# MishaLaskin/vqvae

Hardware: NVIDIA H100
Metric: images/sec VQVAE fwd (enc+VQ+dec) (higher is better)
Workload: dtype tf32

## Files before the change

### vqvae_b200/csrc/vq_backward.cu

```cuda
#include "common.cuh"

namespace {

__global__ void vq_backward_kernel(const float *__restrict__ g_zq, const float *__restrict__ g_loss, const float *__restrict__ z,
                                   const float *__restrict__ E, const long long *__restrict__ idx, long long N, int K, int D,
                                   float beta, float *__restrict__ dz, float *__restrict__ dE) {
    const int d4 = D / 4;
    const long long total = N * d4;
    const float gl = g_loss ? __ldg(g_loss) : 0.f;
    const float c1 = gl * 2.0f / ((float)N * (float)D), c2 = c1 * beta;
    for (long long i = (long long)blockIdx.x * blockDim.x + threadIdx.x; i < total; i += (long long)gridDim.x * blockDim.x) {
        const long long row = i / d4;
        const int c = (int)(i - row * d4);
        long long k = idx[row];
        k = k < 0 ? 0 : (k >= K ? K - 1 : k);
        const float4 zv = __ldg(reinterpret_cast<const float4 *>(z) + i);
        const float4 ev = __ldg(reinterpret_cast<const float4 *>(E + (size_t)k * D) + c);
        float4 g = g_zq ? __ldg(reinterpret_cast<const float4 *>(g_zq) + i) : make_float4(0.f, 0.f, 0.f, 0.f);
        const float4 df = make_float4(zv.x - ev.x, zv.y - ev.y, zv.z - ev.z, zv.w - ev.w);
        g.x = fmaf(c1, df.x, g.x); g.y = fmaf(c1, df.y, g.y); g.z = fmaf(c1, df.z, g.z); g.w = fmaf(c1, df.w, g.w);
        reinterpret_cast<float4 *>(dz)[i] = g;
        float *de = dE + (size_t)k * D + 4 * c;
        atomicAdd(de + 0, -c2 * df.x); atomicAdd(de + 1, -c2 * df.y); atomicAdd(de + 2, -c2 * df.z); atomicAdd(de + 3, -c2 * df.w);
    }
}

}

extern "C" int vqb_vq_backward_f32(const float *g_zq, const float *g_loss, const float *z, const float *codebook,
                                   const int64_t *idx, int64_t N, int K, int D, float beta, float *dz, float *dE, void *stream) {
    if (!z || !codebook || !idx || !dz || !dE) return VQB_ERR_BAD_ARG;
    if (N <= 0 || K <= 0 || D <= 0) return VQB_ERR_BAD_ARG;
    if (D % 4 != 0) return VQB_ERR_UNSUPPORTED;
    const uintptr_t al = reinterpret_cast<uintptr_t>(z) | reinterpret_cast<uintptr_t>(codebook) | reinterpret_cast<uintptr_t>(dz) |
                         reinterpret_cast<uintptr_t>(dE) | reinterpret_cast<uintptr_t>(g_zq);
    if (al & 15) return VQB_ERR_ALIGNMENT;
    cudaStream_t s = (cudaStream_t)stream;
    cudaError_t e = cudaMemsetAsync(dE, 0, sizeof(float) * (size_t)K * D, s);
    if (e != cudaSuccess) return (int)e;
    const long long total = N * (D / 4);
    long long blocks = (total + 255) / 256;
    int dev = 0, sms = 132;
    cudaGetDevice(&dev);
    cudaDeviceGetAttribute(&sms, cudaDevAttrMultiProcessorCount, dev);
    if (blocks > (long long)sms * 16) blocks = (long long)sms * 16;
    vq_backward_kernel<<<(unsigned)blocks, 256, 0, s>>>(g_zq, g_loss, z, codebook, reinterpret_cast<const long long *>(idx), N, K, D, beta,
                                                        dz, dE);
    VQB_COUNT_LAUNCH(1);
    return vqb_cuda_status(cudaGetLastError());
}
```

### vqvae_b200/csrc/wgconv.cu

```cuda
#include "ptx.cuh"
#include "bf16_common.cuh"
#include "wgconv.h"
#include "wgmma.cuh"

namespace {

constexpr int WG_THREADS = 384;
constexpr int WG_MAX_STAGES = 8;
constexpr int A_BYTES = 128 * 128;

struct WgParams {
    const float *bias;
    const void *skip;
    void *out;
    int B, ncols, mid_cols;
    int BW, BH, BN, tiles_x, tiles_y;
    int in_step, out_step, stages;
    int relu, out_bf16;
    int OHg[4], OWg[4], out_py[4], out_px[4], nsteps[4];
    long long out_sn, out_sh, out_sw, out_sc;
    int4 steps[4][WG_MAX_STEPS];
    const void *tail_w;
    const float *tail_bias;
    float *tail_out;
    int tail_cout, tail_relu;
};

constexpr int SC_N = 64;
constexpr int SC_BBYTES = SC_N * 128;

template <bool BF16>
__device__ __forceinline__ void gather_shuffle_weight(uint32_t wres, const void *w, int Cin, int Cout, int nc, int t) {
    const size_t row_bytes = (size_t)Cin * (BF16 ? 2 : 4);
    for (int i = t; i < nc * SC_N * 8; i += 256) {
        const int j = i & 7, r = (i >> 3) % SC_N, c = i / (8 * SC_N);
        const int ph = r >> 4, k = (r >> 2) & 3, co = r & 3;
        const int tap = ((k >> 1) + (ph >> 1)) * 3 + (k & 1) + (ph & 1);
        uint4 v = make_uint4(0u, 0u, 0u, 0u);
        if (co < Cout)
            v = __ldg(reinterpret_cast<const uint4 *>(reinterpret_cast<const unsigned char *>(w) +
                      (size_t)(tap * 16 + ph * Cout + co) * row_bytes + c * 128 + j * 16));
        const uint32_t dst = wres + (uint32_t)(c * SC_BBYTES + r * 128 + ((j ^ (r & 7)) << 4));
        asm volatile("st.shared.v4.b32 [%0], {%1, %2, %3, %4};" ::"r"(dst), "r"(v.x), "r"(v.y), "r"(v.z), "r"(v.w) : "memory");
    }
    ptx::fence_proxy_async();
}

template <int N>
__device__ __forceinline__ void store_tile(const WgParams &p, const float *acc, int ph, int wgi, int gx0, int gy0, int n0,
                                           const void *skip, int relu) {
    const int warp = (threadIdx.x >> 5) & 3, lane = threadIdx.x & 31;
    const int cq = 2 * (lane & 3);
#pragma unroll
    for (int h = 0; h < 2; ++h) {
        const int row = wgi * 64 + warp * 16 + (lane >> 2) + 8 * h;
        const int bw = row % p.BW, bh = (row / p.BW) % p.BH, bn = row / (p.BW * p.BH);
        const int gx = gx0 + bw, gy = gy0 + bh, n = n0 + bn;
        if (gx >= p.OWg[ph] || gy >= p.OHg[ph] || n >= p.B) continue;
        const long long ob = (long long)n * p.out_sn + (long long)(gy * p.out_step + p.out_py[ph]) * p.out_sh +
                             (long long)(gx * p.out_step + p.out_px[ph]) * p.out_sw;
#pragma unroll
        for (int j = 0; j < N / 8; ++j) {
            const int c = 8 * j + cq;
            if (c >= p.ncols) continue;
            float v0 = acc[4 * j + 2 * h], v1 = acc[4 * j + 2 * h + 1];
            if (p.bias) { v0 += __ldg(p.bias + c); v1 += __ldg(p.bias + c + 1); }
            if (p.out_bf16) {
                if (skip) {
                    const __nv_bfloat162 sk = *reinterpret_cast<const __nv_bfloat162 *>(
                        reinterpret_cast<const __nv_bfloat16 *>(skip) + ob + c);
                    v0 += __bfloat162float(sk.x); v1 += __bfloat162float(sk.y);
                }
                if (relu) { v0 = fmaxf(v0, 0.f); v1 = fmaxf(v1, 0.f); }
                *reinterpret_cast<uint32_t *>(reinterpret_cast<__nv_bfloat16 *>(p.out) + ob + c) = pack_bf16(v0, v1);
            } else {
                if (skip) {
                    const float2 sk = *reinterpret_cast<const float2 *>(reinterpret_cast<const float *>(skip) + ob + c);
                    v0 += sk.x; v1 += sk.y;
                }
                if (relu) { v0 = fmaxf(v0, 0.f); v1 = fmaxf(v1, 0.f); }
                *reinterpret_cast<float2 *>(reinterpret_cast<float *>(p.out) + ob + c) = make_float2(v0, v1);
            }
        }
    }
}

template <bool BF16, int N>
__host__ __device__ constexpr int chain_chunks() { return BF16 ? 1 : (N >= 32 ? N / 32 : 1); }

constexpr int TAIL_PHASE_ROWS = 4 * 128;

template <bool BF16, int N, int N2, bool TAIL = false>
__global__ void __launch_bounds__(WG_THREADS, 1)
wgconv_kernel(const __grid_constant__ CUtensorMap tma_in, const __grid_constant__ CUtensorMap tma_w,
              const __grid_constant__ CUtensorMap tma_w2, const __grid_constant__ WgParams p) {
    static_assert(!TAIL || (!BF16 && N == SC_N && N2 == 0), "TAIL: TF32, 64 channels of h, no second GEMM");
    extern __shared__ unsigned char smem_raw[];
    const uint32_t raw = ptx::smem_u32(smem_raw);
    const uint32_t sbase = (raw + 1023u) & ~1023u;
    constexpr int STAGE = A_BYTES + N * 128;
    constexpr int KC2 = chain_chunks<BF16, N>();
    constexpr int HCHUNK = TAIL_PHASE_ROWS * 128;
    const int S = p.stages;
    const uint32_t mid = sbase + (uint32_t)(S * STAGE);
    const uint32_t w2s = mid + (uint32_t)(KC2 * (TAIL ? HCHUNK : A_BYTES));
    const uint32_t bars = mid + (N2 > 0 ? (uint32_t)(KC2 * (A_BYTES + N2 * 128))
                                 : TAIL ? (uint32_t)(KC2 * (HCHUNK + SC_BBYTES)) : 0u);
    auto full = [&](int s) { return bars + 8u * s; };
    auto empty = [&](int s) { return bars + 8u * (WG_MAX_STAGES + s); };
    const uint32_t w2bar = bars + 8u * (2 * WG_MAX_STAGES);

    const int tid = threadIdx.x, warp = tid >> 5, lane = tid & 31;
    const int ph0 = TAIL ? 0 : blockIdx.y, nph = TAIL ? 4 : 1;
    int tile = blockIdx.x;
    const int tx = tile % p.tiles_x; tile /= p.tiles_x;
    const int ty = tile % p.tiles_y; tile /= p.tiles_y;
    const int gx0 = tx * p.BW, gy0 = ty * p.BH, n0 = tile * p.BN;

    if (tid == 0) {
        for (int s = 0; s < S; ++s) { ptx::mbar_init(full(s), 1); ptx::mbar_init(empty(s), 2); }
        ptx::mbar_init(w2bar, 1);
        ptx::fence_mbar_init();
    }
    if (tid == 32) {
        ptx::prefetch_tmap(&tma_in);
        ptx::prefetch_tmap(&tma_w);
        if (N2 > 0) ptx::prefetch_tmap(&tma_w2);
    }
    __syncthreads();
    pdl_launch_dependents();

    if (warp == 0) {
        if constexpr (N2 > 0) {
            if (lane == 0) {
                constexpr int ck = BF16 ? 64 : 32;
                ptx::mbar_expect_tx(w2bar, (uint32_t)(KC2 * N2 * 128));
                for (int c = 0; c < KC2; ++c) ptx::tma_load_2d(w2s + (uint32_t)(c * N2 * 128), &tma_w2, w2bar, c * ck, 0);
            }
        }
        pdl_wait();
        if (lane == 0) {
            int g = 0;
            for (int ph = ph0; ph < ph0 + nph; ++ph)
                for (int i = 0; i < p.nsteps[ph]; ++i, ++g) {
                    const int s = g % S;
                    if (g >= S) ptx::mbar_wait(empty(s), (uint32_t)((g / S - 1) & 1));
                    const int4 st = p.steps[ph][i];
                    const uint32_t dst = sbase + (uint32_t)(s * STAGE);
                    ptx::mbar_expect_tx(full(s), (uint32_t)STAGE);
                    ptx::tma_load_4d(dst, &tma_in, full(s), st.x, gx0 * p.in_step + st.y, gy0 * p.in_step + st.z, n0);
                    ptx::tma_load_2d(dst + A_BYTES, &tma_w, full(s), st.x, st.w);
                }
        }
        return;
    }
    if (warp < 4) return;

    if constexpr (TAIL) gather_shuffle_weight<false>(w2s, p.tail_w, N, p.tail_cout, KC2, tid - 128);
    pdl_wait();
    const int wgi = (warp >> 2) - 1;
    float acc[N / 2];
    int g = 0;
    for (int ph = ph0; ph < ph0 + nph; ++ph) {
#pragma unroll
        for (int i = 0; i < N / 2; ++i) acc[i] = 0.f;
        for (int i = 0; i < p.nsteps[ph]; ++i, ++g) {
            const int s = g % S;
            ptx::mbar_wait(full(s), (uint32_t)((g / S) & 1));
            const uint32_t a = sbase + (uint32_t)(s * STAGE) + (uint32_t)(wgi * 64 * 128), b = sbase + (uint32_t)(s * STAGE) + A_BYTES;
            wg::fence();
#pragma unroll
            for (int kk = 0; kk < 4; ++kk) wg::mma<BF16, N>(acc, wg::desc_sw128(a + 32u * kk), wg::desc_sw128(b + 32u * kk), 1u);
            wg::commit();
            wg::wait<0>();
            wg::fence_regs<N>(acc);
            if ((warp & 3) == 0 && lane == 0) ptx::mbar_arrive(empty(s));
        }
        if constexpr (TAIL) {
            const int wl = warp & 3, cq = 2 * (lane & 3);
#pragma unroll
            for (int h = 0; h < 2; ++h) {
                const int row = wgi * 64 + wl * 16 + (lane >> 2) + 8 * h;
                const int bw = row % p.BW, bh = (row / p.BW) % p.BH, bn = row / (p.BW * p.BH);
                const int hr = (bn * 2 * p.BH + 2 * bh + p.out_py[ph]) * 2 * p.BW + 2 * bw + p.out_px[ph];
                const bool live = gx0 + bw < p.OWg[ph] && gy0 + bh < p.OHg[ph] && n0 + bn < p.B;
                float *o = reinterpret_cast<float *>(p.out) + (long long)(n0 + bn) * p.out_sn +
                           (long long)((gy0 + bh) * p.out_step + p.out_py[ph]) * p.out_sh +
                           (long long)((gx0 + bw) * p.out_step + p.out_px[ph]) * p.out_sw;
#pragma unroll
                for (int j = 0; j < N / 8; ++j) {
                    const int c = 8 * j + cq;
                    float v0 = acc[4 * j + 2 * h], v1 = acc[4 * j + 2 * h + 1];
                    if (p.bias) { v0 += __ldg(p.bias + c); v1 += __ldg(p.bias + c + 1); }
                    if (p.relu) { v0 = fmaxf(v0, 0.f); v1 = fmaxf(v1, 0.f); }
                    const uint32_t addr = mid + (uint32_t)((c >> 5) * HCHUNK + hr * 128 + ((((c & 31) >> 2) ^ (hr & 7)) << 4) + (c & 3) * 4);
                    asm volatile("st.shared.v2.f32 [%0], {%1, %2};" ::"r"(addr), "f"(v0), "f"(v1) : "memory");
                    if (p.out && live) *reinterpret_cast<float2 *>(o + c) = make_float2(v0, v1);
                }
            }
        }
    }

    if constexpr (TAIL) {
        ptx::fence_proxy_async();
        ptx::named_bar_sync(1, 256);
        const int wl = warp & 3, cq = 2 * (lane & 3);
        for (int blk = 4 * wgi; blk < 4 * wgi + 4; ++blk) {
            float y[SC_N / 2];
#pragma unroll
            for (int i = 0; i < SC_N / 2; ++i) y[i] = 0.f;
            wg::fence();
#pragma unroll
            for (int c = 0; c < KC2; ++c) {
                const uint32_t a = mid + (uint32_t)(c * HCHUNK + blk * 64 * 128), b = w2s + (uint32_t)(c * SC_BBYTES);
#pragma unroll
                for (int kk = 0; kk < 4; ++kk) wg::mma<false, SC_N>(y, wg::desc_sw128(a + 32u * kk), wg::desc_sw128(b + 32u * kk), 1u);
            }
            wg::commit();
            wg::wait<0>();
            wg::fence_regs<SC_N>(y);
            ptx::named_bar_sync(2 + wgi, 128);
#pragma unroll
            for (int h = 0; h < 2; ++h) {
                const int q = blk * 64 + wl * 16 + (lane >> 2) + 8 * h;
#pragma unroll
                for (int j = 0; j < SC_N / 8; ++j) {
                    const int c = 8 * j + cq;
                    const uint32_t addr = mid + (uint32_t)((c >> 5) * HCHUNK + q * 128 + (((c & 31) + 2 * q) & 31) * 4);
                    asm volatile("st.shared.v2.f32 [%0], {%1, %2};" ::"r"(addr), "f"(y[4 * j + 2 * h]), "f"(y[4 * j + 2 * h + 1]) : "memory");
                }
            }
        }
        ptx::named_bar_sync(1, 256);
        const int H = p.OHg[0], W = p.OWg[0];
        const int lw = __ffs(4 * p.BW) - 1, lh = __ffs(4 * p.BH) - 1, Cout = p.tail_cout;
        const float *const ys = reinterpret_cast<const float *>(smem_raw + (mid - raw));
        auto yat = [&](int q, int col) {
            return ys[(col >> 5) * (HCHUNK / 4) + q * 32 + (((col & 31) + 2 * q) & 31)];
        };
        const int total = (p.BN * Cout) << (lw + lh);
        for (int e = tid - 128; e < total; e += 256) {
            const int ox = e & (4 * p.BW - 1), oy = (e >> lw) & (4 * p.BH - 1), co = (e >> (lw + lh)) % Cout;
            const int bn = (e >> (lw + lh)) / Cout;
            if (ox >= 4 * W || oy >= 4 * H || n0 + bn >= p.B) continue;
            const int gy = oy >> 1, py = oy & 1, gx = ox >> 1, px = ox & 1;
            const int base = bn * 4 * p.BH * p.BW, col = (py * 2 + px) * 16 + co;
            float t[4];
#pragma unroll
            for (int k = 0; k < 4; ++k) {
                const int hy = gy + (k >> 1) + py - 1, hx = gx + (k & 1) + px - 1;
                t[k] = hy >= 0 && hy < 2 * H && hx >= 0 && hx < 2 * W ? yat(base + hy * 2 * p.BW + hx, col + 4 * k) : 0.f;
            }
            float v = t[0];
            v += t[1];
            v += t[2];
            v += t[3];
            v += p.tail_bias ? __ldg(p.tail_bias + co) : 0.f;
            if (p.tail_relu) v = fmaxf(v, 0.f);
            p.tail_out[(long long)(n0 + bn) * Cout * 16 * H * W + (long long)co * 16 * H * W + oy * 4 * W + ox] = v;
        }
    } else if constexpr (N2 == 0) {
        store_tile<N>(p, acc, ph0, wgi, gx0, gy0, n0, p.skip, p.relu);
    } else {
        const int wl = warp & 3, cq = 2 * (lane & 3);
#pragma unroll
        for (int h = 0; h < 2; ++h) {
            const int row = wgi * 64 + wl * 16 + (lane >> 2) + 8 * h;
            const uint32_t rb = mid + (uint32_t)(row * 128);
            if constexpr (BF16) {
#pragma unroll
                for (int j = 0; j < 8; ++j) {
                    const int c = 8 * j + cq;
                    float v0 = 0.f, v1 = 0.f;
                    if (j < N / 8 && c < p.mid_cols) { v0 = fmaxf(acc[4 * j + 2 * h], 0.f); v1 = fmaxf(acc[4 * j + 2 * h + 1], 0.f); }
                    const uint32_t addr = rb + (uint32_t)(((j ^ (row & 7)) << 4) + cq * 2);
                    asm volatile("st.shared.b32 [%0], %1;" ::"r"(addr), "r"(pack_bf16(v0, v1)) : "memory");
                }
            } else {
#pragma unroll
                for (int j = 0; j < N / 8; ++j) {
                    const int c = 8 * j + cq, piece = (c & 31) >> 2;
                    const float v0 = fmaxf(acc[4 * j + 2 * h], 0.f), v1 = fmaxf(acc[4 * j + 2 * h + 1], 0.f);
                    const uint32_t addr = rb + (uint32_t)((c >> 5) * A_BYTES) + (uint32_t)(((piece ^ (row & 7)) << 4) + (c & 3) * 4);
                    asm volatile("st.shared.v2.f32 [%0], {%1, %2};" ::"r"(addr), "f"(v0), "f"(v1) : "memory");
                }
            }
        }
        ptx::fence_proxy_async();
        ptx::named_bar_sync(1 + wgi, 128);
        ptx::mbar_wait(w2bar, 0);
        float acc2[N2 > 0 ? N2 / 2 : 1];
#pragma unroll
        for (int i = 0; i < N2 / 2; ++i) acc2[i] = 0.f;
        wg::fence();
#pragma unroll
        for (int c = 0; c < KC2; ++c) {
            const uint32_t a = mid + (uint32_t)(c * A_BYTES + wgi * 64 * 128), b = w2s + (uint32_t)(c * N2 * 128);
#pragma unroll
            for (int kk = 0; kk < 4; ++kk)
                wg::mma<BF16, N2>(acc2, wg::desc_sw128(a + 32u * kk), wg::desc_sw128(b + 32u * kk), 1u);
        }
        wg::commit();
        wg::wait<0>();
        wg::fence_regs<N2>(acc2);
        store_tile<N2>(p, acc2, ph0, wgi, gx0, gy0, n0, p.skip, p.relu);
    }
}

int pow2_ceil(int x) {
    int p = 1;
    while (p < x) p <<= 1;
    return p;
}

typedef void (*wg_fn)(CUtensorMap, CUtensorMap, CUtensorMap, WgParams);

template <bool BF16, int N2>
wg_fn pick_n(int N) {
    switch (N) {
        case 16: return wgconv_kernel<BF16, 16, N2>;
        case 32: return wgconv_kernel<BF16, 32, N2>;
        case 64: return wgconv_kernel<BF16, 64, N2>;
        case 128: return wgconv_kernel<BF16, 128, N2>;
        case 256: return N2 == 0 ? wgconv_kernel<BF16, 256, 0> : nullptr;
        default: return nullptr;
    }
}

wg_fn pick(int bf16, int N, int N2) {
    if (!bf16) {
        switch (N2) {
            case 0: return pick_n<false, 0>(N);
            case 64: return (N == 32 || N == 64) ? pick_n<false, 64>(N) : nullptr;
            case 128: return (N == 32 || N == 64) ? pick_n<false, 128>(N) : nullptr;
            default: return nullptr;
        }
    }
    switch (N2) {
        case 0: return pick_n<true, 0>(N);
        case 64: return N <= 64 ? pick_n<true, 64>(N) : nullptr;
        case 128: return N <= 64 ? pick_n<true, 128>(N) : nullptr;
        default: return nullptr;
    }
}

}

int wg_gemm_cols(int ncols) {
    for (int n : {16, 32, 64, 128, 256})
        if (ncols <= n) return n;
    return 0;
}

int launch_wgconv(const WgLaunch &L, cudaStream_t s) {
    if (L.nph < 1 || L.nph > 4 || wg_gemm_cols(L.N) != L.N || L.ncols > L.N) return VQB_ERR_UNSUPPORTED;
    const bool tail = L.tail_out != nullptr;
    if (tail && (L.bf16 || L.N != SC_N || L.ncols != SC_N || L.N2 != 0 || L.nph != 4 || L.out_step != 2 ||
                 L.tail_cout < 1 || L.tail_cout > 4))
        return VQB_ERR_UNSUPPORTED;
    const wg_fn fn = tail ? wgconv_kernel<false, SC_N, 0, true> : pick(L.bf16, L.N, L.N2);
    if (!fn) return VQB_ERR_UNSUPPORTED;
    const int esz = L.bf16 ? 2 : 4, ck = 128 / esz;
    if (L.Cin % ck != 0 || L.w_inner % ck != 0) return VQB_ERR_UNSUPPORTED;
    if (L.out_sc != 1) return VQB_ERR_UNSUPPORTED;
    WgParams q;
    memset(&q, 0, sizeof(q));
    q.bias = L.bias; q.skip = L.skip; q.out = L.out;
    q.B = L.B; q.ncols = L.ncols; q.mid_cols = L.ncols;
    q.in_step = L.in_step; q.out_step = L.out_step;
    q.relu = L.relu; q.out_bf16 = L.out_bf16;
    q.out_sn = L.out_sn; q.out_sh = L.out_sh; q.out_sw = L.out_sw; q.out_sc = L.out_sc;
    q.tail_w = L.tail_w; q.tail_bias = L.tail_bias; q.tail_out = L.tail_out; q.tail_cout = L.tail_cout;
    q.tail_relu = L.tail_relu;
    int maxw = 0, maxh = 0, maxk = 1;
    for (int i = 0; i < L.nph; ++i) {
        if (L.nsteps[i] > WG_MAX_STEPS) return VQB_ERR_UNSUPPORTED;
        q.OHg[i] = L.OHg[i]; q.OWg[i] = L.OWg[i]; q.out_py[i] = L.out_py[i]; q.out_px[i] = L.out_px[i];
        q.nsteps[i] = L.nsteps[i];
        for (int t = 0; t < L.nsteps[i]; ++t) {
            const WgStep &st = L.steps[i][t];
            q.steps[i][t] = make_int4(st.c0, st.dx, st.dy, st.w_row);
        }
        if (L.OWg[i] > maxw) maxw = L.OWg[i];
        if (L.OHg[i] > maxh) maxh = L.OHg[i];
        if (L.nsteps[i] > maxk) maxk = L.nsteps[i];
    }
    if (maxw <= 0 || maxh <= 0) return 0;
    q.BW = pow2_ceil(maxw) < 16 ? pow2_ceil(maxw) : 16;
    q.BH = pow2_ceil(maxh) < 128 / q.BW ? pow2_ceil(maxh) : 128 / q.BW;
    q.BN = 128 / (q.BW * q.BH);
    q.tiles_x = (maxw + q.BW - 1) / q.BW;
    q.tiles_y = (maxh + q.BH - 1) / q.BH;
    const long long tiles_n = (L.B + q.BN - 1) / q.BN;
    if (tail) {
        if (q.tiles_x != 1 || q.tiles_y != 1) return VQB_ERR_UNSUPPORTED;
        for (int i = 0; i < 4; ++i)
            if (L.OHg[i] != maxh || L.OWg[i] != maxw) return VQB_ERR_UNSUPPORTED;
    }

    const CUtensorMapDataType dt = L.bf16 ? CU_TENSOR_MAP_DATA_TYPE_BFLOAT16 : CU_TENSOR_MAP_DATA_TYPE_FLOAT32;
    CUtensorMap tin, tw, tw2;
    const uint64_t dims[4] = {(uint64_t)L.Cin, (uint64_t)L.W, (uint64_t)L.H, (uint64_t)L.B};
    const uint64_t strides[3] = {(uint64_t)L.Cin * esz, (uint64_t)L.W * L.Cin * esz, (uint64_t)L.H * L.W * L.Cin * esz};
    const uint32_t box[4] = {(uint32_t)ck, (uint32_t)(q.BW * L.in_step), (uint32_t)(q.BH * L.in_step), (uint32_t)q.BN};
    const uint32_t es[4] = {1u, (uint32_t)L.in_step, (uint32_t)L.in_step, 1u};
    int rc = vqb_encode_tmap_4d(&tin, dt, L.in, dims, strides, box, es, CU_TENSOR_MAP_SWIZZLE_128B);
    if (rc) return rc;
    rc = vqb_encode_tmap_2d(&tw, dt, L.w, (uint64_t)L.w_inner, (uint64_t)L.w_rows, (uint64_t)L.w_inner * esz, (uint32_t)ck,
                            (uint32_t)L.N, CU_TENSOR_MAP_SWIZZLE_128B);
    if (rc) return rc;
    tw2 = tw;
    int kc2 = 0;
    if (L.N2 > 0) {
        if (L.ncols > 64 || L.w2_inner % ck != 0) return VQB_ERR_UNSUPPORTED;
        if (!L.bf16 && L.ncols != L.N) return VQB_ERR_UNSUPPORTED;
        kc2 = L.bf16 ? 1 : L.N / 32;
        q.mid_cols = L.ncols; q.ncols = L.N2;
        rc = vqb_encode_tmap_2d(&tw2, dt, L.w2, (uint64_t)L.w2_inner, (uint64_t)L.w2_rows, (uint64_t)L.w2_inner * esz, (uint32_t)ck,
                                (uint32_t)L.N2, CU_TENSOR_MAP_SWIZZLE_128B);
        if (rc) return rc;
    }
    const long long grid = (long long)q.tiles_x * q.tiles_y * tiles_n;
    if (grid <= 0 || grid > 0x7fffffffLL) return VQB_ERR_UNSUPPORTED;
    const int stage = A_BYTES + L.N * 128;
    const int fixed = (tail ? (SC_N / 32) * (TAIL_PHASE_ROWS * 128 + SC_BBYTES) : kc2 * (A_BYTES + L.N2 * 128)) +
                      8 * (2 * WG_MAX_STAGES + 1) + 1024;
    auto ring = [&](int budget) {
        const int st = (budget - fixed) / stage;
        return st > WG_MAX_STAGES ? WG_MAX_STAGES : st > maxk ? maxk : st;
    };
    int stages = ring(220 * 1024);
    if (stages < 1) return VQB_ERR_UNSUPPORTED;
    static bool attr_set[64] = {false};
    const int slot = tail ? 24 : (L.bf16 ? 32 : 0) + (L.N2 == 128 ? 16 : L.N2 == 64 ? 8 : 0) + (L.N == 16 ? 0 : L.N == 32 ? 1 : L.N == 64 ? 2 : L.N == 128 ? 3 : 4);
    if (!attr_set[slot]) {
        cudaError_t e = cudaFuncSetAttribute(fn, cudaFuncAttributeMaxDynamicSharedMemorySize, 220 * 1024);
        if (e != cudaSuccess) return (int)e;
        attr_set[slot] = true;
    }
    int dev = 0, sms = 132;
    cudaGetDevice(&dev);
    cudaDeviceGetAttribute(&sms, cudaDevAttrMultiProcessorCount, dev);
    const int shared = ring(113 * 1024);
    if (!tail && grid * L.nph > sms && shared >= (maxk < 3 ? maxk : 3) && shared < stages) {
        int per_sm = 0;
        if (cudaOccupancyMaxActiveBlocksPerMultiprocessor(&per_sm, fn, WG_THREADS, (size_t)(shared * stage + fixed)) ==
                cudaSuccess && per_sm >= 2)
            stages = shared;
    }
    q.stages = stages;
    const int smem = stages * stage + fixed;
    if (cudaError_t le = vqb_launch(fn, dim3((unsigned)grid, tail ? 1u : (unsigned)L.nph), dim3(WG_THREADS), (size_t)smem, s,
                                    tin, tw, tw2, q))
        return (int)le;
    VQB_COUNT_LAUNCH(1);
    return vqb_cuda_status(cudaGetLastError());
}

static bool set_phase(WgLaunch &L, int i, const ConvPhase &ph, int rows_per_tap, bool chunk_outer) {
    const int ck = L.bf16 ? 64 : 32, nc = L.Cin / ck;
    if (ph.ntaps * nc > WG_MAX_STEPS) return false;
    L.in_step = ph.in_step; L.out_step = ph.out_step;
    L.OHg[i] = ph.OHg; L.OWg[i] = ph.OWg; L.out_py[i] = ph.out_py; L.out_px[i] = ph.out_px;
    int n = 0;
    for (int a = 0; a < (chunk_outer ? nc : ph.ntaps); ++a)
        for (int b = 0; b < (chunk_outer ? ph.ntaps : nc); ++b) {
            const int t = chunk_outer ? b : a, c0 = (chunk_outer ? a : b) * ck;
            L.steps[i][n++] = WgStep{c0, ph.tap_dx[t], ph.tap_dy[t], ph.tap_w[t] * rows_per_tap};
        }
    L.nsteps[i] = n;
    return true;
}

static ConvPhase taps3x3(int H, int W) {
    ConvPhase ph;
    conv_phase(conv_geom(3, 3, 1, 1, 0, H, W), 0, ph);
    return ph;
}

bool conv_tc_supported(const ConvLaunch &p) {
    const bool in_nhwc = p.in_sc == 1 && p.in_sw == p.Cin;
    const bool out_nhwc = p.out_sc == 1 && p.out_sw == p.Cout;
    return in_nhwc && out_nhwc && p.Cin % 32 == 0 && p.Cout % 16 == 0 && p.Cout >= 16 && p.Cout <= 256 &&
           (reinterpret_cast<uintptr_t>(p.in) & 15) == 0 && (reinterpret_cast<uintptr_t>(p.out) & 15) == 0 &&
           (p.skip == nullptr || (reinterpret_cast<uintptr_t>(p.skip) & 15) == 0);
}

int launch_conv_tc(WgLaunch &L, const ConvPhase *ph, int nph, int total_taps, bool chunk_outer, cudaStream_t s) {
    if (nph < 1 || nph > 4) return VQB_ERR_UNSUPPORTED;
    L.w_rows = (long long)total_taps * L.ncols; L.w_inner = L.Cin;
    L.N = wg_gemm_cols(L.ncols);
    L.nph = nph;
    for (int i = 0; i < nph; ++i)
        if (!set_phase(L, i, ph[i], L.ncols, chunk_outer)) return VQB_ERR_UNSUPPORTED;
    return launch_wgconv(L, s);
}

constexpr int RS_MID = 32;
constexpr int RS_N = 3 * RS_MID;
constexpr int RS_WBYTES = RS_N * 128;
constexpr int RS_YS = RS_N + 8;
constexpr int RS_MAX_STAGES = 4;
constexpr int TAIL_N = 64;

struct RsParams {
    float *out;
    const float *head_bias, *tail_bias;
    int B, H, W, BW, BH, BN, napps, relu, stages;
    int head_steps, head_stages, tail;
    int4 head[WG_MAX_STEPS];
};

template <int C>
__global__ void __launch_bounds__(WG_THREADS, 1)
res_scatter_kernel(const __grid_constant__ CUtensorMap tma_in, const __grid_constant__ CUtensorMap tma_w1,
                   const __grid_constant__ CUtensorMap tma_w2, const __grid_constant__ CUtensorMap tma_hw,
                   const __grid_constant__ CUtensorMap tma_tw, const __grid_constant__ RsParams p) {
    constexpr int NC = C / 32;
    constexpr int HSTAGE = A_BYTES + C * 128;
    extern __shared__ unsigned char smem_raw[];
    const uint32_t raw = ptx::smem_u32(smem_raw);
    const uint32_t act = (raw + 1023u) & ~1023u;
    const uint32_t ring = act + (uint32_t)(NC * A_BYTES);
    const uint32_t mid = ring + (uint32_t)(p.stages * RS_WBYTES);
    const uint32_t ysm = mid + (uint32_t)A_BYTES;
    const uint32_t w2s = ysm + (uint32_t)(128 * RS_YS * 4);
    const uint32_t bars = w2s + (uint32_t)(C * 128);
    float *const Y = reinterpret_cast<float *>(smem_raw + (ysm - raw));
    auto full = [&](int s) { return bars + 8u * s; };
    auto empty = [&](int s) { return bars + 8u * (RS_MAX_STAGES + s); };
    auto hfull = [&](int s) { return bars + 8u * (2 * RS_MAX_STAGES + s); };
    auto hempty = [&](int s) { return bars + 8u * (3 * RS_MAX_STAGES + s); };
    const uint32_t abar = bars + 8u * (4 * RS_MAX_STAGES), w2bar = abar + 8u, tbar = abar + 16u;
    const int S = p.stages, HS = p.head_stages, nh = p.head_steps;
    const int total = p.napps * 3 * NC;
    const int n0 = blockIdx.x * p.BN;

    const int tid = threadIdx.x, warp = tid >> 5, lane = tid & 31;
    if (tid == 0) {
        for (int s = 0; s < S; ++s) { ptx::mbar_init(full(s), 1); ptx::mbar_init(empty(s), 2); }
        for (int s = 0; s < HS; ++s) { ptx::mbar_init(hfull(s), 1); ptx::mbar_init(hempty(s), 2); }
        ptx::mbar_init(abar, 1);
        ptx::mbar_init(w2bar, 1);
        ptx::mbar_init(tbar, 1);
        ptx::fence_mbar_init();
    }
    if (tid == 32) {
        ptx::prefetch_tmap(&tma_in);
        ptx::prefetch_tmap(&tma_w1);
        ptx::prefetch_tmap(&tma_w2);
        if (nh) ptx::prefetch_tmap(&tma_hw);
        if (p.tail) ptx::prefetch_tmap(&tma_tw);
    }
    __syncthreads();
    pdl_launch_dependents();

    if (warp == 0) {
        auto load_w1 = [&](int g) {
            const int s = g % S;
            ptx::mbar_expect_tx(full(s), (uint32_t)RS_WBYTES);
            ptx::tma_load_2d(ring + (uint32_t)(s * RS_WBYTES), &tma_w1, full(s), (g % NC) * 32, ((g / NC) % 3) * RS_N);
        };
        auto load_weights = [&] {
            ptx::mbar_expect_tx(w2bar, (uint32_t)(C * 128));
            ptx::tma_load_2d(w2s, &tma_w2, w2bar, 0, 0);
            for (int g = 0; g < S; ++g) load_w1(g);
        };
        if (lane == 0 && !nh) load_weights();
        pdl_wait();
        if (lane == 0) {
            if (nh) {
                for (int i = 0; i < nh; ++i) {
                    const int s = i % HS;
                    if (i >= HS) ptx::mbar_wait(hempty(s), (uint32_t)((i / HS - 1) & 1));
                    const int4 st = p.head[i];
                    const uint32_t dst = ring + (uint32_t)(s * HSTAGE);
                    ptx::mbar_expect_tx(hfull(s), (uint32_t)HSTAGE);
                    ptx::tma_load_4d(dst, &tma_in, hfull(s), st.x, st.y, st.z, n0);
                    ptx::tma_load_2d(dst + A_BYTES, &tma_hw, hfull(s), st.x, st.w);
                }
                for (int i = nh > HS ? nh - HS : 0; i < nh; ++i) ptx::mbar_wait(hempty(i % HS), (uint32_t)((i / HS) & 1));
                load_weights();
            } else {
                ptx::mbar_expect_tx(abar, (uint32_t)(NC * A_BYTES));
                for (int c = 0; c < NC; ++c) ptx::tma_load_4d(act + (uint32_t)(c * A_BYTES), &tma_in, abar, c * 32, 0, 0, n0);
            }
            for (int g = S; g < total; ++g) {
                ptx::mbar_wait(empty(g % S), (uint32_t)((g / S - 1) & 1));
                load_w1(g);
            }
            if (p.tail) {
                for (int g = total - S; g < total; ++g) ptx::mbar_wait(empty(g % S), (uint32_t)((g / S) & 1));
                ptx::mbar_expect_tx(tbar, (uint32_t)(NC * TAIL_N * 128));
                for (int c = 0; c < NC; ++c) ptx::tma_load_2d(ring + (uint32_t)(c * TAIL_N * 128), &tma_tw, tbar, c * 32, 0);
            }
        }
        return;
    }
    if (warp < 4) return;

    pdl_wait();
    const int wgi = (warp >> 2) - 1, wl = warp & 3, cw = warp - 4, cq = 2 * (lane & 3);
    const int lbw = __ffs(p.BW) - 1, lbh = __ffs(p.BH) - 1;
    auto act_addr = [&](int row, int c) {
        return act + (uint32_t)((c >> 5) * A_BYTES + row * 128 + ((((c & 31) >> 2) ^ (row & 7)) << 4) + (c & 3) * 4);
    };
    auto live_row = [&](int row) {
        const int bw = row & (p.BW - 1), bh = (row >> lbw) & (p.BH - 1), bn = row >> (lbw + lbh);
        return bw < p.W && bh < p.H && n0 + bn < p.B;
    };
    if (nh) {
        float acc[C / 2];
#pragma unroll
        for (int i = 0; i < C / 2; ++i) acc[i] = 0.f;
        for (int i = 0; i < nh; ++i) {
            const int s = i % HS;
            ptx::mbar_wait(hfull(s), (uint32_t)((i / HS) & 1));
            const uint32_t a = ring + (uint32_t)(s * HSTAGE + wgi * 64 * 128), b = ring + (uint32_t)(s * HSTAGE + A_BYTES);
            wg::fence();
#pragma unroll
            for (int kk = 0; kk < 4; ++kk) wg::mma<false, C>(acc, wg::desc_sw128(a + 32u * kk), wg::desc_sw128(b + 32u * kk), 1u);
            wg::commit();
            wg::wait<0>();
            wg::fence_regs<C>(acc);
            if (wl == 0 && lane == 0) ptx::mbar_arrive(hempty(s));
        }
#pragma unroll
        for (int h = 0; h < 2; ++h) {
            const int row = wgi * 64 + wl * 16 + (lane >> 2) + 8 * h;
            const bool live = live_row(row);
#pragma unroll
            for (int j = 0; j < C / 8; ++j) {
                const int c = 8 * j + cq;
                float v0 = acc[4 * j + 2 * h], v1 = acc[4 * j + 2 * h + 1];
                if (p.head_bias) { v0 += __ldg(p.head_bias + c); v1 += __ldg(p.head_bias + c + 1); }
                v0 = fmaxf(v0, 0.f); v1 = fmaxf(v1, 0.f);
                if (!live) { v0 = 0.f; v1 = 0.f; }
                asm volatile("st.shared.v2.f32 [%0], {%1, %2};" ::"r"(act_addr(row, c)), "f"(v0), "f"(v1) : "memory");
            }
        }
        ptx::fence_proxy_async();
        ptx::named_bar_sync(2 + wgi, 128);
    } else {
        ptx::mbar_wait(abar, 0);
    }
    int g = 0;
    for (int app = 0; app < p.napps; ++app) {
        const bool last = app + 1 == p.napps;
        float m[16];
#pragma unroll
        for (int i = 0; i < 16; ++i) m[i] = 0.f;
#pragma unroll 1
        for (int r = 0; r < 3; ++r) {
            float acc[RS_N / 2];
            for (int c = 0; c < NC; ++c, ++g) {
                const int s = g % S;
                ptx::mbar_wait(full(s), (uint32_t)((g / S) & 1));
                const uint32_t a = act + (uint32_t)(c * A_BYTES + wgi * 64 * 128), b = ring + (uint32_t)(s * RS_WBYTES);
                wg::fence();
#pragma unroll
                for (int kk = 0; kk < 4; ++kk) wg::mma<false, RS_N>(acc, wg::desc_sw128(a + 32u * kk), wg::desc_sw128(b + 32u * kk), (c | kk) != 0);
                wg::commit();
                wg::wait<0>();
                wg::fence_regs<RS_N>(acc);
                if (wl == 0 && lane == 0) ptx::mbar_arrive(empty(s));
            }
            ptx::named_bar_sync(1, 256);
#pragma unroll
            for (int h = 0; h < 2; ++h) {
                float *yr = Y + (wgi * 64 + wl * 16 + (lane >> 2) + 8 * h) * RS_YS + cq;
#pragma unroll
                for (int j = 0; j < RS_N / 8; ++j)
                    *reinterpret_cast<float2 *>(yr + 8 * j) = make_float2(acc[4 * j + 2 * h], acc[4 * j + 2 * h + 1]);
            }
            ptx::named_bar_sync(1, 256);
            const int dy = r - 1;
#pragma unroll
            for (int i = 0; i < 16; ++i) {
                const int q = cw * 16 + i, bw = q & (p.BW - 1), bh = (q >> lbw) & (p.BH - 1);
                const bool row_in = bh + dy >= 0 && bh + dy < p.H;
                const float *yq = Y + (row_in ? q + dy * p.BW : q) * RS_YS + lane;
                const float t0 = row_in && bw > 0 ? yq[-RS_YS] : 0.f;
                const float t1 = row_in ? yq[RS_MID] : 0.f;
                const float t2 = row_in && bw + 1 < p.W ? yq[RS_YS + 2 * RS_MID] : 0.f;
                m[i] += t0;
                m[i] += t1;
                m[i] += t2;
            }
        }
#pragma unroll
        for (int i = 0; i < 16; ++i) {
            const int row = cw * 16 + i;
            const uint32_t addr = mid + (uint32_t)(row * 128 + (((lane >> 2) ^ (row & 7)) << 4) + (lane & 3) * 4);
            asm volatile("st.shared.f32 [%0], %1;" ::"r"(addr), "f"(fmaxf(m[i], 0.f)) : "memory");
        }
        ptx::fence_proxy_async();
        ptx::named_bar_sync(2 + wgi, 128);
        if (app == 0) ptx::mbar_wait(w2bar, 0);
        float acc2[C / 2];
        wg::fence();
#pragma unroll
        for (int kk = 0; kk < 4; ++kk)
            wg::mma<false, C>(acc2, wg::desc_sw128(mid + (uint32_t)(wgi * 64 * 128) + 32u * kk), wg::desc_sw128(w2s + 32u * kk), kk != 0);
        wg::commit();
        wg::wait<0>();
        wg::fence_regs<C>(acc2);
        const int relu = last ? p.relu : 1;
#pragma unroll
        for (int h = 0; h < 2; ++h) {
            const int row = wgi * 64 + wl * 16 + (lane >> 2) + 8 * h;
            const bool live = live_row(row);
#pragma unroll
            for (int j = 0; j < C / 8; ++j) {
                const int c = 8 * j + cq;
                const uint32_t addr = act_addr(row, c);
                float s0, s1;
                asm volatile("ld.shared.v2.f32 {%0, %1}, [%2];" : "=f"(s0), "=f"(s1) : "r"(addr) : "memory");
                float v0 = acc2[4 * j + 2 * h] + s0, v1 = acc2[4 * j + 2 * h + 1] + s1;
                if (relu) { v0 = fmaxf(v0, 0.f); v1 = fmaxf(v1, 0.f); }
                if (!live) { v0 = 0.f; v1 = 0.f; }
                asm volatile("st.shared.v2.f32 [%0], {%1, %2};" ::"r"(addr), "f"(v0), "f"(v1) : "memory");
            }
        }
        if (!last || p.tail) {
            ptx::fence_proxy_async();
            ptx::named_bar_sync(2 + wgi, 128);
        }
    }
    if (p.tail) {
        ptx::mbar_wait(tbar, 0);
        float acc3[TAIL_N / 2];
#pragma unroll
        for (int i = 0; i < TAIL_N / 2; ++i) acc3[i] = 0.f;
        wg::fence();
#pragma unroll
        for (int c = 0; c < NC; ++c) {
            const uint32_t a = act + (uint32_t)(c * A_BYTES + wgi * 64 * 128), b = ring + (uint32_t)(c * TAIL_N * 128);
#pragma unroll
            for (int kk = 0; kk < 4; ++kk) wg::mma<false, TAIL_N>(acc3, wg::desc_sw128(a + 32u * kk), wg::desc_sw128(b + 32u * kk), 1u);
        }
        wg::commit();
        wg::wait<0>();
        wg::fence_regs<TAIL_N>(acc3);
#pragma unroll
        for (int h = 0; h < 2; ++h) {
            const int row = wgi * 64 + wl * 16 + (lane >> 2) + 8 * h;
            const int bw = row & (p.BW - 1), bh = (row >> lbw) & (p.BH - 1), bn = row >> (lbw + lbh);
            if (bw >= p.W || bh >= p.H || n0 + bn >= p.B) continue;
            float *o = p.out + (((long long)(n0 + bn) * p.H + bh) * p.W + bw) * TAIL_N;
#pragma unroll
            for (int j = 0; j < TAIL_N / 8; ++j) {
                const int c = 8 * j + cq;
                float v0 = acc3[4 * j + 2 * h], v1 = acc3[4 * j + 2 * h + 1];
                if (p.tail_bias) { v0 += __ldg(p.tail_bias + c); v1 += __ldg(p.tail_bias + c + 1); }
// ... 325 lines not shown
```

Measured before the change: 1.314 million.

## Share input tiles across sub-pixel phases in tail conv; atomic-free VQ backward

The fused tail transposed-conv kernel now loads each shifted input tile once and applies it to every sub-pixel phase that uses that shift. It keeps four phase accumulators in registers and overlays the intermediate buffer on the stage ring. This cuts repeated TMA loads of the same input, at the cost of higher register pressure and larger stages. Separately, the VQ backward pass replaces the memset plus float atomics for dE with per-code CTAs that scan all indices deterministically; that code only runs in backward, not in the measured forward.

```diff
diff --git a/vqvae_b200/csrc/vq_backward.cu b/vqvae_b200/csrc/vq_backward.cu
--- a/vqvae_b200/csrc/vq_backward.cu
+++ b/vqvae_b200/csrc/vq_backward.cu
@@ -2,27 +2,95 @@
 
 namespace {
 
-__global__ void vq_backward_kernel(const float *__restrict__ g_zq, const float *__restrict__ g_loss, const float *__restrict__ z,
-                                   const float *__restrict__ E, const long long *__restrict__ idx, long long N, int K, int D,
-                                   float beta, float *__restrict__ dz, float *__restrict__ dE) {
+constexpr int VB_CODES = 16;
+constexpr int VB_LANES = 16;
+constexpr int VB_THREADS = VB_CODES * VB_LANES;
+
+__device__ __forceinline__ long long clamp_code(long long k, int K) { return k < 0 ? 0 : (k >= K ? K - 1 : k); }
+
+__device__ __forceinline__ void vq_backward_dz(const float *__restrict__ g_zq, const float *__restrict__ g_loss,
+                                               const float *__restrict__ z, const float *__restrict__ E,
+                                               const long long *__restrict__ idx, long long N, int K, int D,
+                                               float *__restrict__ dz, long long cta, long long nctas) {
     const int d4 = D / 4;
     const long long total = N * d4;
     const float gl = g_loss ? __ldg(g_loss) : 0.f;
-    const float c1 = gl * 2.0f / ((float)N * (float)D), c2 = c1 * beta;
-    for (long long i = (long long)blockIdx.x * blockDim.x + threadIdx.x; i < total; i += (long long)gridDim.x * blockDim.x) {
+    const float c1 = gl * 2.0f / ((float)N * (float)D);
+    for (long long i = cta * blockDim.x + threadIdx.x; i < total; i += nctas * blockDim.x) {
         const long long row = i / d4;
         const int c = (int)(i - row * d4);
-        long long k = idx[row];
-        k = k < 0 ? 0 : (k >= K ? K - 1 : k);
+        const long long k = clamp_code(idx[row], K);
         const float4 zv = __ldg(reinterpret_cast<const float4 *>(z) + i);
         const float4 ev = __ldg(reinterpret_cast<const float4 *>(E + (size_t)k * D) + c);
         float4 g = g_zq ? __ldg(reinterpret_cast<const float4 *>(g_zq) + i) : make_float4(0.f, 0.f, 0.f, 0.f);
         const float4 df = make_float4(zv.x - ev.x, zv.y - ev.y, zv.z - ev.z, zv.w - ev.w);
         g.x = fmaf(c1, df.x, g.x); g.y = fmaf(c1, df.y, g.y); g.z = fmaf(c1, df.z, g.z); g.w = fmaf(c1, df.w, g.w);
         reinterpret_cast<float4 *>(dz)[i] = g;
-        float *de = dE + (size_t)k * D + 4 * c;
-        atomicAdd(de + 0, -c2 * df.x); atomicAdd(de + 1, -c2 * df.y); atomicAdd(de + 2, -c2 * df.z); atomicAdd(de + 3, -c2 * df.w);
     }
+}
+
+__device__ __forceinline__ void vq_backward_de(const float *__restrict__ g_loss, const float *__restrict__ z,
+                                               const float *__restrict__ E, const long long *__restrict__ idx, long long N,
+                                               int K, int D, float beta, float *__restrict__ dE) {
+    __shared__ long long rows[VB_THREADS];
+    __shared__ int codes[VB_THREADS];
+    __shared__ int wsum[VB_THREADS / 32 + 1];
+    const int tid = threadIdx.x, warp = tid >> 5, lane = tid & 31;
+    const int d4 = D / 4;
+    const float gl = g_loss ? __ldg(g_loss) : 0.f;
+    const float c2 = gl * 2.0f / ((float)N * (float)D) * beta;
+    const long long k0 = (long long)blockIdx.x * VB_CODES;
+    const int grp = tid / VB_LANES, gl_lane = tid % VB_LANES;
+    const long long k = k0 + grp;
+    for (int cb = 0; cb < d4; cb += VB_LANES) {
+        const int c = cb + gl_lane;
+        const bool live = k < K && c < d4;
+        const float4 ev = live ? __ldg(reinterpret_cast<const float4 *>(E + (size_t)k * D) + c) : make_float4(0.f, 0.f, 0.f, 0.f);
+        float4 acc = make_float4(0.f, 0.f, 0.f, 0.f);
+        for (long long base = 0; base < N; base += VB_THREADS) {
+            const long long r = base + tid;
+            const long long code = r < N ? clamp_code(__ldg(idx + r), K) - k0 : -1;
+            const bool in = code >= 0 && code < VB_CODES;
+            const unsigned ball = __ballot_sync(0xffffffffu, in);
+            if (lane == 0) wsum[warp] = __popc(ball);
+            __syncthreads();
+            if (tid == 0) {
+                int t = 0;
+                for (int w = 0; w < VB_THREADS / 32; ++w) { const int n = wsum[w]; wsum[w] = t; t += n; }
+                wsum[VB_THREADS / 32] = t;
+            }
+            __syncthreads();
+            if (in) {
+                const int pos = wsum[warp] + __popc(ball & ((1u << lane) - 1u));
+                rows[pos] = r;
+                codes[pos] = (int)code;
+            }
+            __syncthreads();
+            const int n = wsum[VB_THREADS / 32];
+            if (live)
+                for (int j = 0; j < n; ++j) {
+                    if (codes[j] != grp) continue;
+                    const float4 zv = __ldg(reinterpret_cast<const float4 *>(z + (size_t)rows[j] * D) + c);
+                    acc.x = __fadd_rn(acc.x, __fmul_rn(-c2, __fsub_rn(zv.x, ev.x)));
+                    acc.y = __fadd_rn(acc.y, __fmul_rn(-c2, __fsub_rn(zv.y, ev.y)));
+                    acc.z = __fadd_rn(acc.z, __fmul_rn(-c2, __fsub_rn(zv.z, ev.z)));
+                    acc.w = __fadd_rn(acc.w, __fmul_rn(-c2, __fsub_rn(zv.w, ev.w)));
+                }
+            __syncthreads();
+        }
+        if (live) reinterpret_cast<float4 *>(dE + (size_t)k * D)[c] = acc;
+    }
+}
+
+__global__ void __launch_bounds__(VB_THREADS) vq_backward_kernel(const float *__restrict__ g_zq, const float *__restrict__ g_loss,
+                                                                 const float *__restrict__ z, const float *__restrict__ E,
+                                                                 const long long *__restrict__ idx, long long N, int K, int D,
+                                                                 float beta, float *__restrict__ dz, float *__restrict__ dE,
+                                                                 unsigned nde) {
+    if (blockIdx.x < nde)
+        vq_backward_de(g_loss, z, E, idx, N, K, D, beta, dE);
+    else
+        vq_backward_dz(g_zq, g_loss, z, E, idx, N, K, D, dz, blockIdx.x - nde, gridDim.x - nde);
 }
 
 }
@@ -36,16 +104,16 @@
                          reinterpret_cast<uintptr_t>(dE) | reinterpret_cast<uintptr_t>(g_zq);
     if (al & 15) return VQB_ERR_ALIGNMENT;
     cudaStream_t s = (cudaStream_t)stream;
-    cudaError_t e = cudaMemsetAsync(dE, 0, sizeof(float) * (size_t)K * D, s);
-    if (e != cudaSuccess) return (int)e;
     const long long total = N * (D / 4);
     long long blocks = (total + 255) / 256;
     int dev = 0, sms = 132;
     cudaGetDevice(&dev);
     cudaDeviceGetAttribute(&sms, cudaDevAttrMultiProcessorCount, dev);
     if (blocks > (long long)sms * 16) blocks = (long long)sms * 16;
-    vq_backward_kernel<<<(unsigned)blocks, 256, 0, s>>>(g_zq, g_loss, z, codebook, reinterpret_cast<const long long *>(idx), N, K, D, beta,
-                                                        dz, dE);
+    const unsigned nde = (unsigned)((K + VB_CODES - 1) / VB_CODES);
+    vq_backward_kernel<<<nde + (unsigned)blocks, VB_THREADS, 0, s>>>(g_zq, g_loss, z, codebook,
+                                                                    reinterpret_cast<const long long *>(idx), N, K, D, beta,
+                                                                    dz, dE, nde);
     VQB_COUNT_LAUNCH(1);
     return vqb_cuda_status(cudaGetLastError());
 }
diff --git a/vqvae_b200/csrc/wgconv.cu b/vqvae_b200/csrc/wgconv.cu
--- a/vqvae_b200/csrc/wgconv.cu
+++ b/vqvae_b200/csrc/wgconv.cu
@@ -24,7 +24,24 @@
     const float *tail_bias;
     float *tail_out;
     int tail_cout, tail_relu;
+    int tail_nc;
+    int tail_wrow[9][4];
 };
+
+__host__ __device__ constexpr int tail_shift_phases(int si) {
+    const int ry = si / 3 == 0 ? 2 : si / 3 == 1 ? 3 : 1, rx = si % 3 == 0 ? 2 : si % 3 == 1 ? 3 : 1;
+    int m = 0;
+    for (int py = 0; py < 2; ++py)
+        for (int px = 0; px < 2; ++px)
+            if (((ry >> py) & 1) && ((rx >> px) & 1)) m |= 1 << (py * 2 + px);
+    return m;
+}
+template <int SI> struct TailShift { static constexpr int si = SI; };
+template <int SI = 0, typename F>
+__device__ __forceinline__ void for_each_tail_shift(F &&f) {
+    f(TailShift<SI>{});
+    if constexpr (SI + 1 < 9) for_each_tail_shift<SI + 1>(f);
+}
 
 constexpr int SC_N = 64;
 constexpr int SC_BBYTES = SC_N * 128;
@@ -98,20 +115,22 @@
     extern __shared__ unsigned char smem_raw[];
     const uint32_t raw = ptx::smem_u32(smem_raw);
     const uint32_t sbase = (raw + 1023u) & ~1023u;
-    constexpr int STAGE = A_BYTES + N * 128;
+    constexpr int WSLOT = N * 128;
+    constexpr int STAGE = A_BYTES + (TAIL ? 4 : 1) * WSLOT;
     constexpr int KC2 = chain_chunks<BF16, N>();
     constexpr int HCHUNK = TAIL_PHASE_ROWS * 128;
     const int S = p.stages;
-    const uint32_t mid = sbase + (uint32_t)(S * STAGE);
-    const uint32_t w2s = mid + (uint32_t)(KC2 * (TAIL ? HCHUNK : A_BYTES));
-    const uint32_t bars = mid + (N2 > 0 ? (uint32_t)(KC2 * (A_BYTES + N2 * 128))
-                                 : TAIL ? (uint32_t)(KC2 * (HCHUNK + SC_BBYTES)) : 0u);
+    const uint32_t mid = TAIL ? sbase : sbase + (uint32_t)(S * STAGE);
+    const uint32_t w2s = TAIL ? sbase + (uint32_t)(S * STAGE > KC2 * HCHUNK ? S * STAGE : KC2 * HCHUNK)
+                              : mid + (uint32_t)(KC2 * A_BYTES);
+    const uint32_t bars = N2 > 0 ? mid + (uint32_t)(KC2 * (A_BYTES + N2 * 128))
+                          : TAIL ? w2s + (uint32_t)(KC2 * SC_BBYTES) : mid;
     auto full = [&](int s) { return bars + 8u * s; };
     auto empty = [&](int s) { return bars + 8u * (WG_MAX_STAGES + s); };
     const uint32_t w2bar = bars + 8u * (2 * WG_MAX_STAGES);
 
     const int tid = threadIdx.x, warp = tid >> 5, lane = tid & 31;
-    const int ph0 = TAIL ? 0 : blockIdx.y, nph = TAIL ? 4 : 1;
+    const int ph0 = TAIL ? 0 : blockIdx.y, nph = 1;
     int tile = blockIdx.x;
     const int tx = tile % p.tiles_x; tile /= p.tiles_x;
     const int ty = tile % p.tiles_y; tile /= p.tiles_y;
@@ -140,17 +159,37 @@
         }
         pdl_wait();
         if (lane == 0) {
-            int g = 0;
-            for (int ph = ph0; ph < ph0 + nph; ++ph)
-                for (int i = 0; i < p.nsteps[ph]; ++i, ++g) {
-                    const int s = g % S;
-                    if (g >= S) ptx::mbar_wait(empty(s), (uint32_t)((g / S - 1) & 1));
-                    const int4 st = p.steps[ph][i];
-                    const uint32_t dst = sbase + (uint32_t)(s * STAGE);
-                    ptx::mbar_expect_tx(full(s), (uint32_t)STAGE);
-                    ptx::tma_load_4d(dst, &tma_in, full(s), st.x, gx0 * p.in_step + st.y, gy0 * p.in_step + st.z, n0);
-                    ptx::tma_load_2d(dst + A_BYTES, &tma_w, full(s), st.x, st.w);
+            if constexpr (TAIL) {
+                int g = 0;
+                for (int si = 0; si < 9; ++si) {
+                    int nw = 0;
+                    for (int ph = 0; ph < 4; ++ph) nw += p.tail_wrow[si][ph] >= 0;
+                    for (int c = 0; c < p.tail_nc; ++c, ++g) {
+                        const int s = g % S;
+                        if (g >= S) ptx::mbar_wait(empty(s), (uint32_t)((g / S - 1) & 1));
+                        const uint32_t dst = sbase + (uint32_t)(s * STAGE);
+                        ptx::mbar_expect_tx(full(s), (uint32_t)(A_BYTES + nw * WSLOT));
+                        ptx::tma_load_4d(dst, &tma_in, full(s), c * 32, gx0 * p.in_step + 1 - si % 3,
+                                         gy0 * p.in_step + 1 - si / 3, n0);
+                        for (int ph = 0; ph < 4; ++ph)
+                            if (p.tail_wrow[si][ph] >= 0)
+                                ptx::tma_load_2d(dst + (uint32_t)(A_BYTES + ph * WSLOT), &tma_w, full(s), c * 32,
+                                                 p.tail_wrow[si][ph]);
+                    }
                 }
+            } else {
+                int g = 0;
+                for (int ph = ph0; ph < ph0 + nph; ++ph)
+                    for (int i = 0; i < p.nsteps[ph]; ++i, ++g) {
+                        const int s = g % S;
+                        if (g >= S) ptx::mbar_wait(empty(s), (uint32_t)((g / S - 1) & 1));
+                        const int4 st = p.steps[ph][i];
+                        const uint32_t dst = sbase + (uint32_t)(s * STAGE);
+                        ptx::mbar_expect_tx(full(s), (uint32_t)STAGE);
+                        ptx::tma_load_4d(dst, &tma_in, full(s), st.x, gx0 * p.in_step + st.y, gy0 * p.in_step + st.z, n0);
+                        ptx::tma_load_2d(dst + A_BYTES, &tma_w, full(s), st.x, st.w);
+                    }
+            }
         }
         return;
     }
@@ -160,24 +199,40 @@
     pdl_wait();
     const int wgi = (warp >> 2) - 1;
     float acc[N / 2];
-    int g = 0;
-    for (int ph = ph0; ph < ph0 + nph; ++ph) {
-#pragma unroll
-        for (int i = 0; i < N / 2; ++i) acc[i] = 0.f;
-        for (int i = 0; i < p.nsteps[ph]; ++i, ++g) {
-            const int s = g % S;
-            ptx::mbar_wait(full(s), (uint32_t)((g / S) & 1));
-            const uint32_t a = sbase + (uint32_t)(s * STAGE) + (uint32_t)(wgi * 64 * 128), b = sbase + (uint32_t)(s * STAGE) + A_BYTES;
-            wg::fence();
-#pragma unroll
-            for (int kk = 0; kk < 4; ++kk) wg::mma<BF16, N>(acc, wg::desc_sw128(a + 32u * kk), wg::desc_sw128(b + 32u * kk), 1u);
-            wg::commit();
-            wg::wait<0>();
-            wg::fence_regs<N>(acc);
-            if ((warp & 3) == 0 && lane == 0) ptx::mbar_arrive(empty(s));
-        }
-        if constexpr (TAIL) {
-            const int wl = warp & 3, cq = 2 * (lane & 3);
+    if constexpr (TAIL) {
+        float pacc[4][N / 2];
+#pragma unroll
+        for (int ph = 0; ph < 4; ++ph)
+#pragma unroll
+            for (int i = 0; i < N / 2; ++i) pacc[ph][i] = 0.f;
+        int g = 0;
+        for_each_tail_shift([&](auto shift) {
+            constexpr int mask = tail_shift_phases(decltype(shift)::si);
+            for (int c = 0; c < p.tail_nc; ++c, ++g) {
+                const int s = g % S;
+                ptx::mbar_wait(full(s), (uint32_t)((g / S) & 1));
+                const uint32_t a = sbase + (uint32_t)(s * STAGE + wgi * 64 * 128);
+                wg::fence();
+#pragma unroll
+                for (int ph = 0; ph < 4; ++ph) {
+                    if (!((mask >> ph) & 1)) continue;
+                    const uint32_t b = sbase + (uint32_t)(s * STAGE + A_BYTES + ph * WSLOT);
+#pragma unroll
+                    for (int kk = 0; kk < 4; ++kk)
+                        wg::mma<false, N>(pacc[ph], wg::desc_sw128(a + 32u * kk), wg::desc_sw128(b + 32u * kk), 1u);
+                }
+                wg::commit();
+                wg::wait<0>();
+#pragma unroll
+                for (int ph = 0; ph < 4; ++ph)
+                    if ((mask >> ph) & 1) wg::fence_regs<N>(pacc[ph]);
+                if ((warp & 3) == 0 && lane == 0) ptx::mbar_arrive(empty(s));
+            }
+        });
+        ptx::named_bar_sync(1, 256);
+        const int wl = warp & 3, cq = 2 * (lane & 3);
+#pragma unroll
+        for (int ph = 0; ph < 4; ++ph) {
 #pragma unroll
             for (int h = 0; h < 2; ++h) {
                 const int row = wgi * 64 + wl * 16 + (lane >> 2) + 8 * h;
@@ -190,13 +245,31 @@
 #pragma unroll
                 for (int j = 0; j < N / 8; ++j) {
                     const int c = 8 * j + cq;
-                    float v0 = acc[4 * j + 2 * h], v1 = acc[4 * j + 2 * h + 1];
+                    float v0 = pacc[ph][4 * j + 2 * h], v1 = pacc[ph][4 * j + 2 * h + 1];
                     if (p.bias) { v0 += __ldg(p.bias + c); v1 += __ldg(p.bias + c + 1); }
                     if (p.relu) { v0 = fmaxf(v0, 0.f); v1 = fmaxf(v1, 0.f); }
                     const uint32_t addr = mid + (uint32_t)((c >> 5) * HCHUNK + hr * 128 + ((((c & 31) >> 2) ^ (hr & 7)) << 4) + (c & 3) * 4);
                     asm volatile("st.shared.v2.f32 [%0], {%1, %2};" ::"r"(addr), "f"(v0), "f"(v1) : "memory");
                     if (p.out && live) *reinterpret_cast<float2 *>(o + c) = make_float2(v0, v1);
                 }
+            }
+        }
+    } else {
+        int g = 0;
+        for (int ph = ph0; ph < ph0 + nph; ++ph) {
+#pragma unroll
+            for (int i = 0; i < N / 2; ++i) acc[i] = 0.f;
+            for (int i = 0; i < p.nsteps[ph]; ++i, ++g) {
+                const int s = g % S;
+                ptx::mbar_wait(full(s), (uint32_t)((g / S) & 1));
+                const uint32_t a = sbase + (uint32_t)(s * STAGE) + (uint32_t)(wgi * 64 * 128), b = sbase + (uint32_t)(s * STAGE) + A_BYTES;
+                wg::fence();
+#pragma unroll
+                for (int kk = 0; kk < 4; ++kk) wg::mma<BF16, N>(acc, wg::desc_sw128(a + 32u * kk), wg::desc_sw128(b + 32u * kk), 1u);
+                wg::commit();
+                wg::wait<0>();
+                wg::fence_regs<N>(acc);
+                if ((warp & 3) == 0 && lane == 0) ptx::mbar_arrive(empty(s));
             }
         }
     }
@@ -350,6 +423,31 @@
     for (int n : {16, 32, 64, 128, 256})
         if (ncols <= n) return n;
     return 0;
+}
+
+static bool tail_shift_table(const WgLaunch &L, int nc, int ck, int wrow[9][4]) {
+    int next[4] = {0, 0, 0, 0};
+    for (int si = 0; si < 9; ++si) {
+        const int dy = 1 - si / 3, dx = 1 - si % 3;
+        int mask = 0;
+        for (int ph = 0; ph < 4; ++ph) {
+            wrow[si][ph] = -1;
+            if (next[ph] >= L.nsteps[ph]) continue;
+            const WgStep &st = L.steps[ph][next[ph]];
+            if (st.dy == dy && st.dx == dx) { wrow[si][ph] = st.w_row; mask |= 1 << ph; }
+        }
+        if (mask != tail_shift_phases(si)) return false;
+        for (int c = 0; c < nc; ++c)
+            for (int ph = 0; ph < 4; ++ph) {
+                if (wrow[si][ph] < 0) continue;
+                if (next[ph] >= L.nsteps[ph]) return false;
+                const WgStep &st = L.steps[ph][next[ph]++];
+                if (st.c0 != c * ck || st.dy != dy || st.dx != dx || st.w_row != wrow[si][ph]) return false;
+            }
+    }
+    for (int ph = 0; ph < 4; ++ph)
+        if (next[ph] != L.nsteps[ph]) return false;
+    return true;
 }
 
 int launch_wgconv(const WgLaunch &L, cudaStream_t s) {
@@ -393,9 +491,12 @@
     q.tiles_y = (maxh + q.BH - 1) / q.BH;
     const long long tiles_n = (L.B + q.BN - 1) / q.BN;
     if (tail) {
-        if (q.tiles_x != 1 || q.tiles_y != 1) return VQB_ERR_UNSUPPORTED;
+        if (q.tiles_x != 1 || q.tiles_y != 1 || L.in_step != 1) return VQB_ERR_UNSUPPORTED;
         for (int i = 0; i < 4; ++i)
             if (L.OHg[i] != maxh || L.OWg[i] != maxw) return VQB_ERR_UNSUPPORTED;
+        q.tail_nc = L.Cin / ck;
+        if (!tail_shift_table(L, q.tail_nc, ck, q.tail_wrow)) return VQB_ERR_UNSUPPORTED;
+        maxk = 9 * q.tail_nc;
     }
 
     const CUtensorMapDataType dt = L.bf16 ? CU_TENSOR_MAP_DATA_TYPE_BFLOAT16 : CU_TENSOR_MAP_DATA_TYPE_FLOAT32;
@@ -422,9 +523,9 @@
     }
     const long long grid = (long long)q.tiles_x * q.tiles_y * tiles_n;
     if (grid <= 0 || grid > 0x7fffffffLL) return VQB_ERR_UNSUPPORTED;
-    const int stage = A_BYTES + L.N * 128;
-    const int fixed = (tail ? (SC_N / 32) * (TAIL_PHASE_ROWS * 128 + SC_BBYTES) : kc2 * (A_BYTES + L.N2 * 128)) +
-                      8 * (2 * WG_MAX_STAGES + 1) + 1024;
+    const int stage = A_BYTES + (tail ? 4 : 1) * L.N * 128;
+    const int fixed = (tail ? (SC_N / 32) * SC_BBYTES : kc2 * (A_BYTES + L.N2 * 128)) + 8 * (2 * WG_MAX_STAGES + 1) + 1024;
+    const int overlay = tail ? (SC_N / 32) * TAIL_PHASE_ROWS * 128 : 0;
     auto ring = [&](int budget) {
         const int st = (budget - fixed) / stage;
         return st > WG_MAX_STAGES ? WG_MAX_STAGES : st > maxk ? maxk : st;
@@ -449,7 +550,7 @@
             stages = shared;
     }
     q.stages = stages;
-    const int smem = stages * stage + fixed;
+    const int smem = (stages * stage > overlay ? stages * stage : overlay) + fixed;
     if (cudaError_t le = vqb_launch(fn, dim3((unsigned)grid, tail ? 1u : (unsigned)L.nph), dim3(WG_THREADS), (size_t)smem, s,
                                     tin, tw, tw2, q))
         return (int)le;
```

New measurement: 1.333 million (median of 6 runs). +1.4%, better.
